# rsutormin/KmerGutsJava

Hardware: AMD Instinct MI355X
Metric: amino-acid residues/sec scanned (and hits/sec) on 1 Gbp synthetic, 1/2/4/8 MI355X (higher is better)
Workload: dtype int64; 1 GPU; 1 Gbp contig mix (0.5 kbp..1.024 Mbp, uniform ACGT) on 1 GPU, 6-frame translate + 8-mer lookup vs 1400303159-slot signature table (33.6 GB, load 0.50), -m 5 -g 200; total_bp_rank0=1000000000, contigs_rank0=6351, total_bp_all_ranks=1000000000, num_sigs=1400303159, residues_rank0=1999974596, residues_all_ranks=1999974596, hits_rank0=36744843, hits_all_ranks=36744843, calls_rank0=4, parallelism=contig shards x1, table replicated

## Files before the change

### kmergutsjava_amd/csrc/kg_host_plan.hpp

```cpp
#pragma once

namespace {


template <typename T, T V, T... Vs, typename F>
void dispatch(T x, F &&f)
{
    if constexpr (sizeof...(Vs) == 0) f(std::integral_constant<T, V>{});
    else if (x == V) f(std::integral_constant<T, V>{});
    else dispatch<T, Vs...>(x, f);
}

struct BatchPlan {
    std::vector<uint32_t> ibase;
    uint64_t nblocks = 0, windows = 0, residues = 0;
    uint64_t n_rows = 0, n_cont = 0;
    int64_t longest = 0;
};

template <bool AA>
int plan_batch(const int64_t *offsets, int64_t n_seqs, BatchPlan &b)
{
    constexpr uint32_t PER = AA ? 1 : 6;
    b.ibase.resize((size_t)n_seqs + 1);
    for (int64_t k = 0; k < n_seqs; k++) {
        int64_t L = offsets[k + 1] - offsets[k];
        if (L < 0) return fail(KG_ERR_ARG, "offsets must be non-decreasing");
        b.longest = std::max(b.longest, L);
        if (L > 0xFFFFFFF0ll) return fail(KG_ERR_LIMIT, "a single sequence longer than 2^32-16 characters");
        b.ibase[(size_t)k] = (uint32_t)b.nblocks;
        uint64_t nb;
        if (AA) {
            uint64_t nwin = L >= 9 ? (uint64_t)L - 8 : 0;
            b.windows += nwin;
            b.residues += (uint64_t)L;
            nb = (nwin + kg::kAaWinPerBlock - 1) / kg::kAaWinPerBlock;
        } else {
            uint64_t npos = L >= 24 ? (uint64_t)L - 23 : 0;
            b.windows += 2 * npos;
            for (int f = 0; f < 3; f++)
                if (L - f >= 3) b.residues += 2 * (uint64_t)((L - f) / 3);
            nb = (npos + kg::kDnaPosPerBlock - 1) / kg::kDnaPosPerBlock;
        }
        b.nblocks += nb;
        if (b.nblocks > 0x7FFFFFFFull / PER) return fail(KG_ERR_LIMIT, "batch too large: more than 2^31-1 window rows; split the batch");
    }
    b.ibase[(size_t)n_seqs] = (uint32_t)b.nblocks;
    if (b.windows > 0xFFFFFF00ull) return fail(KG_ERR_LIMIT, "batch too large: more than 2^32-256 windows; split the batch");
    b.n_rows = b.nblocks * PER;
    b.n_cont = (uint64_t)n_seqs * PER;
    return KG_OK;
}

uint64_t bucket_count(uint64_t limit, uint32_t shift) { return (limit + (1ull << shift) - 1) >> shift; }

struct PartPlan {
    bool applicable = false;
    uint32_t shift = 0, buckets = 0;
    uint32_t n_chunks = 0;
    std::vector<uint64_t> clo;
    std::vector<int64_t> cseq;
    uint64_t max_chunk = 0;
    uint32_t n_wg = 0, cap = 0;
    uint64_t n_regions = 0;
    uint32_t ovf_cap = 0;
    uint32_t gshift = 10, groups_stride = 0;
    size_t next_stride = 0;
    size_t scatter_lds = 0;
    bool use_bidx = false, part_counters = false, prog_index = false;
    uint32_t probe_grid = 0, index_grid = 0, verify_grid = 0, lowc_grid = 0, ovf_grid = 0, order_grid = 0;
    uint32_t scatter_prio = 0, index_prio = 0, verify_prio = 0, index_r = 1, probe_grab = 0;
    uint32_t flush_list = 0;
    uint64_t list_slack = 0, ucap = 0, ccap = 0;
    uint32_t n_os = 0;
    bool early_totals = false, place_staged = false, debug = false;
};

template <bool AA>
int plan_partition(const kg_table *t, const BatchPlan &b, bool progress, bool counters_req, PartPlan &pl)
{
    constexpr uint32_t PER = AA ? 1 : 6;
    const uint64_t nblocks = b.nblocks;
    uint32_t shift = env_knob("KG_PART_SHIFT", 21u, 4u, 31u);
    const uint64_t qmax = (uint64_t)KG_MAX_ENCODED / (uint64_t)t->num_sigs + 1;
    while (shift > 4 && qmax >= (1ull << (32 - shift))) shift--;
    while (bucket_count(t->limit, shift) > (uint64_t)kg::kMaxBuckets) shift++;
    while (kg::scatter_lds_bytes<AA>((uint32_t)bucket_count(t->limit, shift)) > 160u * 1024) shift++;
    const bool fits = shift < 32 && qmax < (1ull << (32 - shift)) && nblocks <= (1ull << 23) && t->m35 != 0 &&
                      t->limit < (1ull << 32) - 64;
    const uint32_t mode = env_u32("KG_PARTITION", 2u);
    const bool worth = t->limit >= (64ull << 20) && b.windows >= (1ull << 27);
    if (!(fits && nblocks > 0 && (mode == 1 || (mode == 2 && worth)))) return KG_OK;
    pl.shift = shift;
    pl.buckets = (uint32_t)bucket_count(t->limit, shift);

    constexpr uint32_t WIN = AA ? 64u : 384u;
    uint32_t want = env_u32("KG_PART_CHUNKS", 4u);
    if (want < 1) want = 1;
    if (want > kMaxChunks) want = kMaxChunks;
    if (getenv("KG_PART_MIN_CHUNK_BLOCKS")) {
        const uint64_t min_chunk = std::max(1u, env_u32("KG_PART_MIN_CHUNK_BLOCKS", 600000u));
        while (want > 1 && nblocks / want < min_chunk) want--;
    } else {
        const uint32_t by_size = nblocks < 450000 ? 1u : std::max(2u, (uint32_t)std::lround(std::sqrt((double)nblocks / 325000.0)));
        want = std::min(want, std::max(1u, by_size));
    }
    pl.clo.push_back(0); pl.cseq.push_back(0);
    std::vector<double> cum;
    if (const char *tp = getenv("KG_PART_TAPER")) {
        double acc = 0;
        for (const char *q = tp; *q;) {
            char *endp = nullptr;
            const double v = strtod(q, &endp);
            if (endp == q) break;
            acc += v; cum.push_back(acc);
            q = *endp == ',' ? endp + 1 : endp;
        }
        if (cum.size() >= 2 && cum.size() <= kMaxChunks && acc > 0) { for (auto &x : cum) x /= acc; want = (uint32_t)cum.size(); }
        else cum.clear();
    }
    for (uint32_t c = 1; c < want; c++) {
        const uint64_t target = cum.empty() ? nblocks * c / want : (uint64_t)((double)nblocks * cum[c - 1]);
        const auto it = std::lower_bound(b.ibase.begin(), b.ibase.end(), (uint32_t)target);
        const uint64_t cut = *it;
        if (cut > pl.clo.back() && cut < nblocks) { pl.clo.push_back(cut); pl.cseq.push_back((int64_t)(it - b.ibase.begin())); }
    }
    pl.clo.push_back(nblocks); pl.cseq.push_back((int64_t)b.ibase.size() - 1);
    pl.n_chunks = (uint32_t)pl.clo.size() - 1;
    for (uint32_t c = 0; c < pl.n_chunks; c++) pl.max_chunk = std::max(pl.max_chunk, pl.clo[c + 1] - pl.clo[c]);
    const uint64_t max_chunk = pl.max_chunk;
    const uint64_t chunk_blocks = (max_chunk + kg::kScatterWaves - 1) / kg::kScatterWaves * kg::kScatterWaves;
    const double max_frac = (double)max_chunk / (double)nblocks;
    uint32_t n_wg = env_knob("KG_PART_WGS", 256u, 1u, kMaxGrid);
    if ((uint64_t)n_wg * kg::kScatterWaves > chunk_blocks) n_wg = (uint32_t)((chunk_blocks + kg::kScatterWaves - 1) / kg::kScatterWaves);
    const uint64_t blocks_per_wg = ((chunk_blocks + (uint64_t)n_wg * kg::kScatterWaves - 1) / ((uint64_t)n_wg * kg::kScatterWaves)) * kg::kScatterWaves;
    const double mean = (double)blocks_per_wg * WIN / (double)pl.buckets * (env_u32("KG_PART_SLACK", 100u) / 100.0);
    const uint64_t cap64 = ((uint64_t)(mean + 6.0 * std::sqrt(mean) + 32.0) + 15) / 16 * 16;
    if (cap64 >= (1ull << 24) || (uint64_t)pl.buckets * n_wg >= (1ull << 24)) return KG_OK;
    pl.n_wg = n_wg;
    pl.cap = (uint32_t)cap64;
    pl.n_regions = (uint64_t)pl.buckets * n_wg;
    pl.ovf_cap = env_u32("KG_PART_OVF_GROUPS", (uint32_t)std::min<uint64_t>(1u << 23, std::max<uint64_t>(65536, pl.n_regions * pl.cap / 16 / 8)));
    while (pl.gshift < 12 && ((max_chunk * PER) >> pl.gshift) + 2 > 8192) pl.gshift++;
    pl.groups_stride = (uint32_t)(((max_chunk * PER) >> pl.gshift) + 2);
    if (pl.groups_stride > kg::kMaxGroups) return fail(KG_ERR_LIMIT, "a chunk of the batch holds more than 2^26 window rows");
    pl.next_stride = std::max<size_t>((size_t)pl.buckets + 8, 256);
    pl.use_bidx = t->d_bidx != nullptr && !counters_req && env_u32("KG_BIDX", 1u) != 0;
    pl.part_counters = (counters_req || progress) && !pl.use_bidx;
    pl.prog_index = progress && pl.use_bidx;
    pl.scatter_lds = kg::scatter_lds_bytes<AA>(pl.buckets);
    pl.flush_list = env_knob("KG_SCATTER_FLUSH_LIST", kg::scatter_flush_list_max<AA>(), 1u, kg::scatter_flush_list_max<AA>());
    pl.probe_grid = env_knob("KG_PROBE_GRID", 256u * 8u, 8u, kMaxGrid, 8u);
    pl.index_grid = env_knob("KG_INDEX_GRID", 256u * 4u, 8u, kMaxGrid, 8u);
    pl.scatter_prio = std::min(3u, env_u32("KG_SCATTER_PRIO", 1u));
    pl.index_prio = std::min(3u, env_u32("KG_INDEX_PRIO", 2u));
    pl.verify_prio = std::min(3u, env_u32("KG_VERIFY_PRIO", pl.n_chunks == 1 ? 2u : 0u));
    uint32_t index_r = env_u32("KG_INDEX_R", 0u);
    if (index_r == 0) index_r = mean * 0.7 >= 640.0 ? 1u : mean * 0.7 >= 320.0 ? 2u : 4u;
    if (index_r != 1 && index_r != 2) index_r = 4;
    while (index_r > 1 && (n_wg % index_r != 0 || kg::kIndexN % index_r != 0)) index_r /= 2;
    pl.index_r = index_r;
    pl.verify_grid = env_knob("KG_VERIFY_GRID", 256u * 2u, 1u, kMaxGrid);
    pl.lowc_grid = env_knob("KG_LOWC_GRID", 256u, 1u, kMaxGrid);
    pl.ovf_grid = env_knob("KG_OVF_GRID", 256u, 1u, kMaxGrid);
    pl.list_slack = (uint64_t)(std::max(std::max(pl.probe_grid, pl.index_grid), pl.verify_grid) + 64) * 4 * kg::kUChunk + 4096;
    pl.ucap = ((uint64_t)((double)b.windows * t->stage_ratio * max_frac) + pl.list_slack + kg::kUChunk - 1) / kg::kUChunk * kg::kUChunk;
    pl.ccap = ((uint64_t)((double)b.windows * (t->stage_ratio * 1.25 + 0.03) * max_frac) + pl.list_slack + kg::kUChunk - 1) /
              kg::kUChunk * kg::kUChunk;
    if (test_hook("KG_TEST_TINY_LISTS")) pl.ucap = pl.ccap = kg::kUChunk;
    const uint32_t grab_unit = 256u * (uint32_t)std::max(kg::kProbeN, kg::kIndexN);
    pl.probe_grab = env_knob("KG_PROBE_GRAB", pl.cap, grab_unit, 1u << 24, grab_unit);
    pl.n_os = pl.n_chunks < 2 ? 0u : std::min(env_u32("KG_ORDER_STREAMS", 0u), kMaxOrderStreams);
    pl.early_totals = pl.n_os == 0 && env_u32("KG_EARLY_TOTALS", 1u) != 0;
    pl.order_grid = env_knob("KG_ORDER_GRID", 256u * 3u, 1u, kMaxGrid);
    pl.place_staged = pl.gshift == 10 && env_u32("KG_PLACE_STAGED", 1u) != 0;
    pl.debug = getenv("KG_DEBUG") != nullptr;
    pl.applicable = true;
    return KG_OK;
}

struct DirectPlan {
    uint32_t scan_grid, stage_chunk;
    const uint32_t *d_hbits;
    uint32_t rpg;
    uint64_t stage_cap;
};

template <bool AA>
DirectPlan plan_direct(const kg_table *t, const BatchPlan &b, bool counters)
{
    DirectPlan pl;
    pl.scan_grid = env_knob("KG_SCAN_GRID", 256u * 8u, 1u, kMaxGrid);
    pl.stage_chunk = env_knob("KG_STAGE_CHUNK", 256u, 1u, 1u << 12);
    const uint32_t filter_mode = env_u32("KG_DIRECT_FILTER", 1u);
    pl.d_hbits = (counters || filter_mode == 0 || (filter_mode == 1 && t->limit <= (4ull << 20))) ? nullptr : t->d_hbits;
    pl.rpg = AA ? 1u : env_u32("KG_SCAN_RPG", pl.d_hbits ? 6u : 3u);
    if (pl.rpg != 1 && pl.rpg != 2 && pl.rpg != 3 && pl.rpg != 6) pl.rpg = 3;
    pl.stage_cap = (uint64_t)((double)b.windows * t->stage_ratio) + 4096 + (uint64_t)pl.scan_grid * kg::kWavesPerWG * pl.stage_chunk;
    if (pl.stage_cap > 0xFFFFFF00ull) pl.stage_cap = 0xFFFFFF00ull;
    if (test_hook("KG_TEST_TINY_LISTS")) pl.stage_cap = 256;
    return pl;
}

struct AggPlan {
    uint32_t pshift;
    bool pieces_on;
    uint32_t agg_pairs;
};

AggPlan plan_aggregate()
{
    AggPlan pl;
    pl.pshift = std::min(20u, std::max(6u, env_u32("KG_AGG_BLOCK_SHIFT", 9u)));
    pl.pieces_on = env_u32("KG_AGG_PIECES", 1u) != 0;
    pl.agg_pairs = env_u32("KG_AGG_PAIRS", 1u);
    return pl;
}

}
```

### kmergutsjava_amd/csrc/kg_partition.hpp

```cpp
#pragma once

#include "kg_device.hpp"

namespace kg {

constexpr int kMaxBuckets = 1024;
#ifndef KG_PROBE_N
#define KG_PROBE_N 4
#endif
#ifndef KG_SCATTER_WPE
#define KG_SCATTER_WPE 5
#endif
#ifndef KG_TAG_WPE
#define KG_TAG_WPE 8
#endif
#if KG_SCATTER_WPE
#define KG_SCATTER_REGS __attribute__((amdgpu_waves_per_eu(KG_SCATTER_WPE)))
#else
#define KG_SCATTER_REGS
#endif
#if KG_TAG_WPE
#define KG_TAG_REGS __attribute__((amdgpu_waves_per_eu(KG_TAG_WPE)))
#else
#define KG_TAG_REGS
// ... 229 lines not shown
                        lowc = true;
                        if (RG != ROWS) wave_sync();
                    }
                }
            }
        }
        n_valid += nv;
        uint32_t spins = 0;
        if (insert_prio) set_wave_prio(insert_prio);
        for (;;) {
            uint32_t at[RG], old[RG];
#pragma unroll
            for (int r = 0; r < RG; r++)
                at[r] = (pend & (1u << r)) ? atomicAdd(&cnt[bk[r]], 1u) : kGroup;
#pragma unroll
            for (int r = 0; r < RG; r++) {
                old[r] = 0;
                if (at[r] < kGroup) {
                    buf[(size_t)bk[r] * kGroup + at[r]] = e[r];
                    __builtin_amdgcn_fence(__ATOMIC_RELEASE, "wavefront");
                    old[r] = atomicAdd(&written[bk[r]], 1u);
                }
            }
            __builtin_amdgcn_fence(__ATOMIC_ACQUIRE, "wavefront");
#pragma unroll
            for (int r = 0; r < RG; r++) pend &= ~((uint32_t)(at[r] < kGroup) << r);
            uint32_t at_max = at[0];
#pragma unroll
            for (int r = 1; r < RG; r++) at_max = max(at_max, at[r]);
            uint32_t left = 0;
            auto list_rows = [&](auto again) -> uint32_t {
                uint32_t n = 0;
#pragma unroll
                for (int r = 0; r < RG; r++) {
                    const bool own = decltype(again)::value ? ((left >> r) & 1u) != 0 : (old[r] & 15u) == 15u;
                    const unsigned long long m = __ballot(own);
                    if (m) {
                        const uint32_t rank = __builtin_amdgcn_mbcnt_hi((uint32_t)(m >> 32), __builtin_amdgcn_mbcnt_lo((uint32_t)m, n));
                        if (own && rank < list_cap) {
                            const uint32_t g = decltype(again)::value ? (written[bk[r]] >> 4) - 1u : old[r] >> 4;
                            flist[rank] = (min(g, gcap) << 10) | bk[r];
                            if (decltype(again)::value) left &= ~(1u << r);
                        }
                        n += (uint32_t)__popcll(m);
                    }
                }
                return n;
            };
            uint32_t n_own = list_rows(std::false_type{});
            if (__builtin_expect(n_own > list_cap, 0)) {
                uint32_t k = 0;
#pragma unroll
                for (int r = 0; r < RG; r++) {
                    const bool own = (old[r] & 15u) == 15u;
                    const unsigned long long m = __ballot(own);
                    const uint32_t rank = __builtin_amdgcn_mbcnt_hi((uint32_t)(m >> 32), __builtin_amdgcn_mbcnt_lo((uint32_t)m, k));
                    if (own && rank >= list_cap) left |= 1u << r;
                    k += (uint32_t)__popcll(m);
                }
            }
            while (n_own) {
                const uint32_t n_list = min(n_own, list_cap);
                wave_sync();
                for (uint32_t p0 = 0; p0 < n_list; p0 += 8) {
                    const uint32_t want = p0 + ((uint32_t)lane >> 3), sub = (uint32_t)lane & 7u;
                    if (want < n_list) {
                        const uint32_t d = flist[want];
                        const uint32_t fb = d & (uint32_t)(kMaxBuckets - 1), g = d >> 10;
                        const ulonglong2 v = *reinterpret_cast<const ulonglong2 *>(buf + (size_t)fb * kGroup + 2 * sub);
                        __builtin_amdgcn_fence(__ATOMIC_RELEASE, "wavefront");
                        if (sub == 0) cnt[fb] = 0;
                        const bool full = g >= gcap;
                        if (!full) {
                            unsigned char *to = reinterpret_cast<unsigned char *>(ent) + (mul24_wide(__umul24(fb, n_wg) + w, cap) << 3);
                            store_entry_pair(reinterpret_cast<uint64_t *>(to + ((g << 7) | (sub << 4))), v);
                        }
                        if (__builtin_expect(__ballot(full) != 0, 0)) scatter_overflow_octets(cold, full, fb, v.x, v.y);
                    }
                }
                wave_sync();
                if (__builtin_expect(n_own <= list_cap, 1)) break;
                n_own = list_rows(std::true_type{});
            }
            if (!__ballot(pend != 0)) break;
            {
                const int rp = pend ? __builtin_ctz(pend) : 0;
                uint32_t pb = bk[0];
#pragma unroll
                for (int r = 1; r < RG; r++)
                    if (rp == r) pb = bk[r];
                for (uint32_t polls = 0; polls < 64; polls++) {
                    if (__ballot(pend != 0 && __hip_atomic_load(&cnt[pb], __ATOMIC_RELAXED, __HIP_MEMORY_SCOPE_WORKGROUP) < kGroup)) break;
                    __builtin_amdgcn_s_sleep(2);
                }
            }
            if (__builtin_expect(++spins > (1u << 20) || __ballot(at_max >= (1u << 28)), 0)) {
                scatter_protocol_failure(cold);
                break;
            }
        }
        if (insert_prio) set_wave_prio(0);
        }
    }
    __syncthreads();
    const uint32_t per_wave = (n_buckets + kScatterWaves - 1) / kScatterWaves;
    const uint32_t b_end = min((uint32_t)(wave + 1) * per_wave, n_buckets);
    for (uint32_t b0 = (uint32_t)wave * per_wave; b0 < b_end; b0 += 64) {
        const uint32_t b = b0 + (uint32_t)lane;
        const uint32_t wr = b < b_end ? written[b] : 0u;
        const uint32_t c = wr & 15u, g = wr >> 4;
        unsigned long long dst = kDstNone;
        bool to_ovf = false;
        if (c > 0) {
            for (uint32_t k = c; k < kGroup; k++) buf[(size_t)b * kGroup + k] = kEntInvalid;
            if (g < gcap) dst = ((uint64_t)b * n_wg + w) * cap + ((uint64_t)g << 4);
            else to_ovf = true;
        }
        const unsigned long long movf = __ballot(to_ovf);
        if (movf) dst = scatter_overflow_groups(cold, movf, to_ovf, b, dst);
        unsigned long long m = __ballot(dst != kDstNone);
        wave_sync();
        while (m) {
            int src_lane = -1;
            unsigned long long mm = m;
#pragma unroll
            for (int o = 0; o < 8; o++) {
                const int ln = mm ? __builtin_ctzll(mm) : -1;
                if (mm) mm &= mm - 1;
                if ((lane >> 3) == o) src_lane = ln;
            }
            m = mm;
            const int sl = src_lane < 0 ? 0 : src_lane;
            const uint32_t fb = (uint32_t)__shfl((int)b, sl);
            const unsigned long long to = __shfl(dst, sl);
            if (src_lane >= 0) {
                const uint32_t sub = (uint32_t)lane & 7u;
                const ulonglong2 v = *reinterpret_cast<const ulonglong2 *>(buf + (size_t)fb * kGroup + 2 * sub);
                if (__builtin_expect((to & kDstOvf) != 0, 0)) {
                    if (to != kDstDropped) scatter_store_overflow(cold, to, sub, v.x, v.y);
                } else {
                    store_entry_pair(ent + to + 2 * sub, v);
                }
            }
        }
    }
    for (uint32_t b = threadIdx.x; b < n_buckets; b += blockDim.x)
        fill[(uint64_t)b * n_wg + w] = min((written[b] + 15u) >> 4, gcap) << 4;
    for (int off = 32; off > 0; off >>= 1) n_valid += __shfl_down(n_valid, off);
    unsigned long long *ctr = cold->ctr;
    if (lane == 0 && n_valid) atomicAdd(&ctr[0], (unsigned long long)n_valid);
    if constexpr (SHORT) flush_ran_off(ran_off, ctr, lane);
}

constexpr int kLowcWaves = 4;
template <bool AA>
__global__ __launch_bounds__(64 * kLowcWaves) void lowc_blocks_kernel(
    const uint8_t *__restrict__ seq, const BlockDesc *__restrict__ blocks, const uint32_t *__restrict__ lowc_cursor,
    const uint32_t *__restrict__ lowc_blocks, uint64_t limit, uint32_t num_sigs, uint32_t m35, uint32_t shift, uint32_t n_regions,
    uint32_t cap, uint64_t *__restrict__ ent, uint32_t *__restrict__ fill, uint32_t *ovf_cursor, uint32_t ovf_cap,
    uint32_t *__restrict__ ovf_bucket, uint64_t *__restrict__ ovf_ent, unsigned long long *ctr, Progress *prog)
{
    constexpr int ROWS = AA ? 1 : 6;
    __shared__ typename WaveLds<AA>::type lds[kLowcWaves];
    __shared__ typename WaveLds<AA>::tables enc_tables;
    const int lane = threadIdx.x & 63, wave = threadIdx.x >> 6;
    typename WaveLds<AA>::type &l = lds[wave];
    const uint32_t n_list = *lowc_cursor;
    if (n_list == 0) return;
    encode_init<AA>(enc_tables, threadIdx.x, blockDim.x);
    __syncthreads();
    const uint32_t limit32 = limit < 0xFFFFFFFFull ? (uint32_t)limit : 0xFFFFFFFFu;
    unsigned long long n_valid = 0;
    bool ran_off = false;
    uint32_t pool_at = 0, pool_end = 0;
    auto pool_flush = [&]() {
        for (uint32_t g = pool_at + ((uint32_t)lane >> 4); g < pool_end && g < ovf_cap; g += 4) {
            if ((lane & 15) == 0) ovf_bucket[g] = 0;
            ovf_ent[(uint64_t)g * kGroup + ((uint32_t)lane & 15u)] = kEntInvalid;
        }
        pool_at = pool_end;
    };
    auto ovf_groups = [&](uint32_t lead, uint32_t ng) -> uint64_t * {
        if (pool_end - pool_at < ng) {
            pool_flush();
            const uint32_t want = ng > 32u ? ng : 32u;
            uint32_t g0 = 0;
            if (lane == 0) g0 = atomicAdd(ovf_cursor, want);
            g0 = (uint32_t)__builtin_amdgcn_readfirstlane((int)g0);
            pool_at = g0; pool_end = g0 + want;
        }
        const uint32_t g = pool_at;
        pool_at += ng;
        if (g + ng > ovf_cap) return nullptr;
        if ((uint32_t)lane < ng) ovf_bucket[g + lane] = lead;
        return ovf_ent + (uint64_t)g * kGroup;
    };
    for (uint32_t i = blockIdx.x * kLowcWaves + (uint32_t)wave; i < n_list; i += gridDim.x * kLowcWaves) {
        const uint32_t it = (uint32_t)__builtin_amdgcn_readfirstlane((int)lowc_blocks[i]);
        const BlockDesc bd = blocks[it];
        encode_block<AA>(l, enc_tables, seq, bd, lane);
        const uint32_t region_w = it % n_regions;
        for (int r = 0; r < ROWS; r++) {
            uint32_t hi, lo, q;
            bool valid = row_halves<AA>(l, r, lane, bd, &hi, &lo);
            const uint32_t slot = split_fast(hi, lo, num_sigs, m35, &q);
            if (valid) n_valid++;
            if (valid && slot >= limit32) { ran_off = true; if (prog) progress_note_beyond(prog, slot); }
            bool pend = valid && slot < limit32;
            const uint32_t bkt = slot >> shift;
            const uint64_t e = ((uint64_t)window_key<AA>(bd, it, r, lane) << 32) | ((q << shift) | (slot & ((1u << shift) - 1u)));
            for (int pass = 0; pass < 4; pass++) {
                const unsigned long long mp = __ballot(pend);
                if (__popcll(mp) < 16) break;
                const uint32_t lead = (uint32_t)__builtin_amdgcn_readlane((int)bkt, __builtin_ctzll(mp));
                const bool mine = pend && bkt == lead;
                const unsigned long long same = __ballot(mine);
                const uint32_t n = (uint32_t)__popcll(same);
                if (n < 8) break;
                const uint32_t rank = (uint32_t)__popcll(same & ((1ull << lane) - 1ull));
                const uint64_t region = (uint64_t)lead * n_regions + region_w;
                uint32_t rel = cap;
                if (lane == 0 && *const_cast<volatile uint32_t *>(&fill[region]) < cap) rel = atomicAdd(&fill[region], n);
                rel = (uint32_t)__builtin_amdgcn_readfirstlane((int)rel);
                if (rel + n <= cap) {
                    if (mine) ent[region * cap + rel + rank] = e;
                } else {
                    if (rel < cap && (uint32_t)lane < cap - rel) ent[region * cap + rel + lane] = kEntInvalid;
                    const uint32_t npad = (n + kGroup - 1) & ~(kGroup - 1);
                    uint64_t *dst = ovf_groups(lead, npad / kGroup);
                    if (dst) {
                        if (mine) dst[rank] = e;
                        if ((uint32_t)lane < npad - n) dst[n + lane] = kEntInvalid;
                    }
                }
                if (mine) pend = false;
            }
            if (pend) {
                const uint64_t region = (uint64_t)bkt * n_regions + region_w;
                const uint32_t rel = atomicAdd(&fill[region], 1u);
                if (rel < cap) { ent[region * cap + rel] = e; pend = false; }
            }
            for (;;) {
                const unsigned long long mp = __ballot(pend);
                if (!mp) break;
                const uint32_t lead = (uint32_t)__builtin_amdgcn_readlane((int)bkt, __builtin_ctzll(mp));
                const bool mine = pend && bkt == lead;
                const unsigned long long same = __ballot(mine);
                const uint32_t n = (uint32_t)__popcll(same);
                const uint32_t npad = (n + kGroup - 1) & ~(kGroup - 1);
                const uint32_t rank = (uint32_t)__popcll(same & ((1ull << lane) - 1ull));
                uint64_t *dst = ovf_groups(lead, npad / kGroup);
                if (dst) {
                    if (mine) dst[rank] = e;
                    if ((uint32_t)lane < npad - n) dst[n + lane] = kEntInvalid;
                }
                if (mine) pend = false;
            }
        }
        wave_sync();
    }
    pool_flush();
    for (int off = 32; off > 0; off >>= 1) n_valid += __shfl_down(n_valid, off);
    if (lane == 0 && n_valid) atomicAdd(&ctr[0], n_valid);
    flush_ran_off(ran_off, ctr, lane);
}

struct UListState { unsigned long long base; uint32_t used; bool have; };

template <bool AA, int N, bool COUNTERS>
__device__ __forceinline__ void probe_entries(const TableView &tab, uint32_t b, uint32_t shift, const uint64_t (&e)[N],
                                              kg_hit *__restrict__ ulist, uint32_t *__restrict__ chunk_used,
                                              unsigned long long *cursor, uint64_t ulist_cap, UListState &u,
                                              unsigned long long &ctr_slots, bool &ran_off, int lane, Progress *prog)
{
    uint64_t val[N], slot[N];
    bool valid[N];
    uint32_t id[N], fp[N];
#pragma unroll
    for (int k = 0; k < N; k++) {
        valid[k] = e[k] != kEntInvalid;
        const uint32_t low = (uint32_t)e[k];
        id[k] = (uint32_t)(e[k] >> 32);
        slot[k] = ((uint64_t)b << shift) | (low & ((1u << shift) - 1u));
        val[k] = (uint64_t)(low >> shift) * tab.num_sigs + slot[k];
        fp[k] = tag_qs(low >> shift, slot[k]);
    }
    Payload pay[N];
    unsigned long long ctr_dummy = 0;
    uint32_t fslot[N];
#pragma unroll
    for (int k = 0; k < N; k++) fslot[k] = 0;
    const uint32_t foundm = probe_n<N, COUNTERS>(tab, val, slot, fp, valid, pay, ctr_dummy, ctr_slots, ran_off, COUNTERS ? prog : nullptr,
                                                 COUNTERS ? fslot : nullptr);
    uint32_t cnt[N], rank[N], total = 0;
#pragma unroll
    for (int k = 0; k < N; k++) {
        const bool f = (foundm >> k) & 1u;
        const unsigned long long m = __ballot(f);
        cnt[k] = (uint32_t)__popcll(m);
        rank[k] = (uint32_t)__popcll(m & ((1ull << lane) - 1ull));
        total += cnt[k];
    }
    if (total) {
        if (u.used + total > kUChunk) {
            if (lane == 0 && u.have && u.base + kUChunk <= ulist_cap) chunk_used[u.base / kUChunk] = u.used;
            unsigned long long nb = 0;
            if (lane == 0) nb = atomicAdd(cursor, (unsigned long long)kUChunk);
            nb = ((unsigned long long)__builtin_amdgcn_readfirstlane((uint32_t)(nb >> 32)) << 32) |
                 (unsigned long long)__builtin_amdgcn_readfirstlane((uint32_t)nb);
            u.base = nb; u.used = 0; u.have = true;
        }
        if (u.base + kUChunk <= ulist_cap) {
            uint32_t at = u.used;
#pragma unroll
            for (int k = 0; k < N; k++) {
                if ((foundm >> k) & 1u) {
                    kg_hit h;
                    h.container = id[k];
                    h.from0InProt = (int32_t)fslot[k];
                    h.oI = pay[k].oI; h.avgOffFromEnd = pay[k].avg; h.fI = pay[k].fI; h.functionWt = pay[k].wt;
                    ulist[u.base + at + rank[k]] = h;
                }
                at += cnt[k];
            }
        }
        u.used += total;
    }
}

struct CandRec { uint32_t home, quo, id, walked; };
constexpr uint32_t kWalkOn = 0x80000000u;
constexpr uint32_t kScanOn = 0x40000000u;
constexpr uint32_t kWalkedMask = 0x3FFFFFFFu;
static_assert(sizeof(CandRec) == 16, "CandRec must be 16 bytes");

__device__ __forceinline__ unsigned long long chunk_reserve(UListState &u, uint32_t total, uint32_t *__restrict__ chunk_used,
                                                            unsigned long long *cursor, uint64_t cap, int lane)
{
    if (u.used + total > kUChunk) {
        if (lane == 0 && u.have && u.base + kUChunk <= cap) chunk_used[u.base / kUChunk] = u.used;
        unsigned long long nb = 0;
        if (lane == 0) nb = atomicAdd(cursor, (unsigned long long)kUChunk);
        nb = ((unsigned long long)__builtin_amdgcn_readfirstlane((uint32_t)(nb >> 32)) << 32) |
             (unsigned long long)__builtin_amdgcn_readfirstlane((uint32_t)nb);
        u.base = nb; u.used = 0; u.have = true;
    }
    const unsigned long long at = u.base + u.used;
    u.used += total;
    return u.base + kUChunk <= cap ? at : ~0ull;
}

__device__ __forceinline__ void chunk_finish(const UListState &u, uint32_t *__restrict__ chunk_used, uint64_t cap, int lane)
{
    if (lane == 0 && u.have && u.base + kUChunk <= cap) chunk_used[u.base / kUChunk] = u.used;
}

template <bool COUNTERS>
__global__ __launch_bounds__(256) KG_TAG_REGS void bucket_tag_kernel(
    const uint8_t *__restrict__ tags, uint64_t limit, uint64_t num_sigs, const uint64_t *__restrict__ ent,
    const uint32_t *__restrict__ fill, uint32_t n_regions, uint32_t cap, uint32_t n_buckets, uint32_t shift,
    uint32_t grab ,
    uint32_t *next_region ,
    CandRec *__restrict__ cand, uint32_t *__restrict__ cand_used, unsigned long long *cand_cursor, uint64_t cand_cap,
// ... 109 lines not shown
        const CandRec out = stage[(uint32_t)lane < sfill ? lane : 0];
        const unsigned long long at = chunk_reserve(u, sfill, cand_used, cand_cursor, cand_cap, lane);
        if (at != ~0ull && (uint32_t)lane < sfill) stream_store16(cand + at + (uint32_t)lane, &out);
    }
    chunk_finish(u, cand_used, cand_cap, lane);
    flush_ran_off(ran_off, ctr, lane);
    if (COUNTERS) {
        for (int off = 32; off > 0; off >>= 1) ctr_slots += __shfl_down(ctr_slots, off);
        if (lane == 0) atomicAdd(&ctr[1], ctr_slots);
    }
}

template <int N, int R, bool EXACT, bool PROG = false>
__global__ __launch_bounds__(256) KG_TAG_REGS void bucket_index_kernel(
    const uint8_t *__restrict__ bidx, uint32_t tail_start,
    const uint64_t *__restrict__ ent, const uint32_t *__restrict__ fill, uint32_t n_regions , uint32_t cap, uint32_t n_buckets,
    uint32_t shift, uint32_t grab ,
    uint32_t *next_region ,
    CandRec *__restrict__ cand, uint32_t *__restrict__ cand_used, unsigned long long *cand_cursor, uint64_t cand_cap,
    unsigned long long *ctr, uint32_t prio , Progress *prog )
{
    static_assert(N % R == 0, "R must divide N");
    constexpr int PER = N / R;
    __shared__ uint32_t s_region;
    __shared__ uint32_t s_lut[256];
    __shared__ __attribute__((aligned(16))) CandRec s_stage[4][kStageFlush + 64];
    CandRec *stage = s_stage[__builtin_amdgcn_readfirstlane((int)(threadIdx.x >> 6))];
    uint32_t sfill = 0;
    const int lane = threadIdx.x & 63;
    bool ran_off = false;
    UListState u;
    u.base = 0; u.used = kUChunk; u.have = false;
    s_lut[threadIdx.x] = bidx_decode(threadIdx.x);
    if (prio) set_wave_prio(prio);

    const uint32_t kGrab = grab;
    const uint32_t grabs_per_region = (cap + kGrab - 1) / kGrab;
    const uint32_t n_grabs = (n_regions / R) * grabs_per_region;
    const uint32_t xg = blockIdx.x & 7u;
    const uint32_t n_tickets = xg < n_buckets ? ((n_buckets - xg + 7u) / 8u) * n_grabs : 0u;
    constexpr uint32_t all_walk = EXACT ? 0u : kBidxInexact;
    for (;;) {
        __syncthreads();
        if (threadIdx.x == 0) s_region = atomicAdd(&next_region[xg * 32u], 1u);
        __syncthreads();
        const uint32_t tk = s_region;
        if (tk >= n_tickets) break;
        const uint32_t b = xg + 8u * (tk / n_grabs), g = tk % n_grabs;
        const uint32_t w = (g / grabs_per_region) * R, g0 = (g % grabs_per_region) * kGrab;
        uint32_t fraw[R], n[R], nmax = cap;
#pragma unroll
        for (int r = 0; r < R; r++) { fraw[r] = fill[(uint64_t)b * n_regions + w + r]; n[r] = cap; }
        const uint64_t *src = ent + ((uint64_t)b * n_regions + w) * cap;
        const uint32_t smask = (1u << shift) - 1u, bbase = b << shift;
        uint32_t d_lo = 0, d_hi = 0, pmin = ~0u, pmax1 = 0;
        if (PROG) {
            const uint64_t s0 = (uint64_t)b << shift, s1 = (((uint64_t)b + 1) << shift) - 1;
#pragma unroll
            for (int k = 1; k <= 10; k++) { d_lo += prog->lo[k] <= s0 ? 1u : 0u; d_hi += prog->lo[k] <= s1 ? 1u : 0u; }
        }
        for (uint32_t c0 = g0; c0 < nmax && c0 < g0 + kGrab; c0 += 256u * PER) {
            uint64_t ev[N];
#pragma unroll
            for (int k = 0; k < N; k++) {
                const int r = k / PER;
                const uint32_t i = c0 + (uint32_t)(k % PER) * 256u + threadIdx.x;
                ev[k] = i < n[r] ? __builtin_nontemporal_load(src + (uint64_t)r * cap + i) : kEntInvalid;
            }
            if (c0 == g0) {
                nmax = 0;
#pragma unroll
                for (int r = 0; r < R; r++) {
                    uint32_t f = fraw[r];
                    asm volatile("; fill first used here" : "+s"(f));
                    n[r] = min(f, cap);
                    nmax = max(nmax, n[r]);
                }
            }
            uint32_t code[N], vmask = 0;
#pragma unroll
            for (int k = 0; k < N; k++) {
                if (c0 + (uint32_t)(k % PER) * 256u + threadIdx.x >= n[k / PER]) ev[k] = kEntInvalid;
                code[k] = 0;
                if (ev[k] != kEntInvalid) {
                    vmask |= 1u << k;
                    code[k] = bidx[bbase | ((uint32_t)ev[k] & smask)];
                }
            }
            uint32_t candm = 0, walkm = 0, wd[N];
#pragma unroll
            for (int k = 0; k < N; k++) wd[k] = s_lut[code[k]];
#pragma unroll
            for (int k = 0; k < N; k++) {
                const uint32_t q = (uint32_t)ev[k] >> shift;
                const uint32_t c = EXACT ? q : q % kBidxClasses;
                const uint32_t listed = (wd[k] >> c) & 1u;
                candm |= listed << k;
                walkm |= (listed & ((wd[k] | all_walk) >> 31)) << k;
                ran_off = ran_off || (((vmask >> k) & 1u) && !listed && (bbase | ((uint32_t)ev[k] & smask)) >= tail_start);
            }
            if (PROG) {
                if (d_lo == d_hi) {
#pragma unroll
                    for (int k = 0; k < N; k++) {
                        const uint32_t h = bbase | ((uint32_t)ev[k] & smask);
                        if ((vmask >> k) & 1u) pmin = min(pmin, h);
                        if (((vmask & ~candm) >> k) & 1u) pmax1 = max(pmax1, h + 1u);
                    }
                } else {
                    for (int k = 0; k < N; k++)
                        if ((vmask >> k) & 1u) progress_note_home(prog, d_lo, d_hi, bbase | ((uint32_t)ev[k] & smask), (candm >> k) & 1u);
                }
            }
#pragma unroll
            for (int k = 0; k < N; k++) {
                const unsigned long long m = __ballot((candm >> k) & 1u);
                if (!m) continue;
                if ((candm >> k) & 1u) {
                    CandRec c;
                    c.home = bbase | ((uint32_t)ev[k] & smask); c.quo = (uint32_t)ev[k] >> shift;
                    c.id = (uint32_t)(ev[k] >> 32); c.walked = ((walkm >> k) & 1u) ? kWalkOn : kScanOn;
                    stage[sfill + (uint32_t)__popcll(m & ((1ull << lane) - 1ull))] = c;
                }
                sfill += (uint32_t)__popcll(m);
                while (sfill >= kStageFlush) {
                    wave_sync();
                    const unsigned long long at = chunk_reserve(u, kStageFlush, cand_used, cand_cursor, cand_cap, lane);
                    if ((uint32_t)lane < kStageFlush) {
                        const ulonglong2 out = *reinterpret_cast<const ulonglong2 *>(stage + lane);
                        if (at != ~0ull) stream_store16(cand + at + (uint32_t)lane, &out);
                    }
                    sfill -= kStageFlush;
                    wave_sync();
                    if ((uint32_t)lane < sfill) {
                        const ulonglong2 rest = *reinterpret_cast<const ulonglong2 *>(stage + kStageFlush + lane);
                        *reinterpret_cast<ulonglong2 *>(stage + lane) = rest;
                    }
                    wave_sync();
                }
            }
        }
        if (PROG && d_lo == d_hi) progress_note_homes(prog, d_lo, pmin, pmax1);
    }
    if (sfill) {
        wave_sync();
        const CandRec out = stage[(uint32_t)lane < sfill ? lane : 0];
        const unsigned long long at = chunk_reserve(u, sfill, cand_used, cand_cursor, cand_cap, lane);
        if (at != ~0ull && (uint32_t)lane < sfill) stream_store16(cand + at + (uint32_t)lane, &out);
    }
    chunk_finish(u, cand_used, cand_cap, lane);
    flush_ran_off(ran_off, ctr, lane);
}

template <bool AA, bool COUNTERS, bool PROG = false>
__global__ __launch_bounds__(256) void verify_kernel(
    const uint8_t *__restrict__ entries, const uint8_t *__restrict__ tags, uint64_t limit, uint64_t num_sigs, uint64_t magic,
    const CandRec *__restrict__ cand, const uint32_t *__restrict__ cand_used, const unsigned long long *cand_cursor,
    uint64_t cand_cap, kg_hit *__restrict__ ulist, uint32_t *__restrict__ chunk_used, unsigned long long *cursor,
    uint64_t ulist_cap, unsigned long long *ctr, Progress *prog ,
    uint32_t prio )
{
    const int lane = threadIdx.x & 63;
    const uint32_t wave_global = __builtin_amdgcn_readfirstlane(blockIdx.x * 4 + (threadIdx.x >> 6));
    const uint32_t n_waves = gridDim.x * 4;
    if (prio) set_wave_prio(prio);
    TableView tab;
    tab.entries = entries; tab.tags = tags; tab.limit = limit; tab.num_sigs = num_sigs; tab.magic = magic; tab.m35 = 0;
    const unsigned long long cur = *cand_cursor;
    const uint32_t n_chunks = (uint32_t)((cur < cand_cap ? cur : cand_cap) / kUChunk);
    unsigned long long ctr_slots = 0;
    bool ran_off = false;
    UListState u;
    u.base = 0; u.used = kUChunk; u.have = false;
    for (uint32_t c = wave_global; c < n_chunks; c += n_waves) {
        const uint32_t used = cand_used[c];
        for (uint32_t k0 = 0; k0 < used; k0 += 64) {
            const bool act = k0 + (uint32_t)lane < used;
            CandRec r;
            r.home = 0; r.quo = 0; r.id = 0; r.walked = 0;
            if (act) {
                const kg_u32x4 cv = __builtin_nontemporal_load(reinterpret_cast<const kg_u32x4 *>(cand + (uint64_t)c * kUChunk + k0 + lane));
                r.home = cv.x; r.quo = cv.y; r.id = cv.z; r.walked = cv.w;
            }
            const uint64_t quo = r.quo, home = r.home;
            const uint64_t val = quo * num_sigs + home;
            uint64_t s = home + (r.walked & kWalkedMask);
            bool found = false;
            Entry e;
            e.key = 0; e.oI = e.avg = e.fI = 0; e.wt = 0.f;
            if (act && (r.walked & kScanOn)) {
#if KG_SCAN_FULL
                if (s < limit) {
                    const uint64_t s1 = s + 1 < limit ? s + 1 : s, s2 = s + 2 < limit ? s + 2 : s;
                    const Entry e0 = load_entry(tab, s);
                    const uint2 k1 = *reinterpret_cast<const uint2 *>(tab.entries + s1 * 24);
                    const uint2 k2 = *reinterpret_cast<const uint2 *>(tab.entries + s2 * 24);
                    const uint32_t vlo = (uint32_t)val, vhi = (uint32_t)(val >> 32);
                    if (e0.key == (int64_t)val) { found = true; e = e0; }
                    else if (s + 1 < limit && k1.x == vlo && k1.y == vhi) { found = true; s += 1; e = load_entry(tab, s); }
                    else if (s + 2 < limit && k2.x == vlo && k2.y == vhi) { found = true; s += 2; e = load_entry(tab, s); }
                    else s += 3;
                }
#endif
                while (!found) {
                    if (s >= limit) { s = limit; ran_off = true; break; }
                    const uint64_t s1 = s + 1 < limit ? s + 1 : s, s2 = s + 2 < limit ? s + 2 : s;
                    const uint2 k0 = *reinterpret_cast<const uint2 *>(tab.entries + s * 24);
                    const uint2 k1 = *reinterpret_cast<const uint2 *>(tab.entries + s1 * 24);
                    const uint2 k2 = *reinterpret_cast<const uint2 *>(tab.entries + s2 * 24);
                    const uint32_t vlo = (uint32_t)val, vhi = (uint32_t)(val >> 32);
                    if (k0.x == vlo && k0.y == vhi) found = true;
                    else if (s + 1 < limit && k1.x == vlo && k1.y == vhi) { found = true; s += 1; }
                    else if (s + 2 < limit && k2.x == vlo && k2.y == vhi) { found = true; s += 2; }
                    if (found) { e = load_entry(tab, s); break; }
                    s += 3;
                }
                if (COUNTERS) {
                    ctr_slots += (s < limit ? s + 1 : limit) - home;
                    if (prog) progress_note_walk(prog, home, s, limit);
                } else if (PROG) {
                    progress_note_walk(prog, home, s, limit);
                }
            } else if (act) {
                if (!(r.walked & kWalkOn)) {
                    e = load_entry(tab, s);
                    found = e.key == (int64_t)val;
                    if (!found) s += 1;
                }
                if (!found) {
                    const uint32_t f = tag_qs(quo, home);
                    for (;;) {
                        if (s >= limit) { s = limit; ran_off = true; break; }
                        const Tags16 x = load_tags(tab.tags + s);
                        bool emp;
                        const int i = first_stop(x, f, &emp);
                        if (i == 16) { s += 16; continue; }
                        s += (uint64_t)i;
                        if (emp) { if (s >= limit) ran_off = true; break; }
                        e = load_entry(tab, s);
                        if (e.key == (int64_t)val) { found = true; break; }
                        s += 1;
                    }
                }
                if (COUNTERS) {
                    ctr_slots += (s < limit ? s + 1 : limit) - home;
                    if (prog) progress_note_walk(prog, home, s, limit);
                } else if (PROG) {
                    progress_note_walk(prog, home, s, limit);
                }
            }
            const unsigned long long m = __ballot(found);
            const uint32_t total = (uint32_t)__popcll(m);
            if (total) {
                const unsigned long long at = chunk_reserve(u, total, chunk_used, cursor, ulist_cap, lane);
                if (at != ~0ull && found) {
                    kg_hit h;
                    h.container = r.id;
                    h.from0InProt = (int32_t)(uint32_t)s;
                    h.oI = e.oI; h.avgOffFromEnd = e.avg; h.fI = e.fI; h.functionWt = e.wt;
                    stream_store_hit(ulist + at + (uint32_t)__popcll(m & ((1ull << lane) - 1ull)), h);
                }
            }
        }
    }
    chunk_finish(u, chunk_used, ulist_cap, lane);
    flush_ran_off(ran_off, ctr, lane);
    if (COUNTERS) {
        for (int off = 32; off > 0; off >>= 1) ctr_slots += __shfl_down(ctr_slots, off);
        if (lane == 0) atomicAdd(&ctr[1], ctr_slots);
    }
}

template <bool AA, bool COUNTERS, bool PROG = false>
__global__ __launch_bounds__(256) void overflow_probe_kernel(
    const uint8_t *__restrict__ entries, const uint8_t *__restrict__ tags, uint64_t limit, uint64_t num_sigs, uint64_t magic,
    const uint32_t *__restrict__ ovf_bucket, const uint64_t *__restrict__ ovf_ent, const uint32_t *__restrict__ ovf_cursor,
    uint32_t ovf_cap, uint32_t shift, kg_hit *__restrict__ ulist, uint32_t *__restrict__ chunk_used, unsigned long long *cursor, uint64_t ulist_cap,
    unsigned long long *ctr, Progress *prog)
{
    const int lane = threadIdx.x & 63;
    const uint32_t wave_global = __builtin_amdgcn_readfirstlane(blockIdx.x * 4 + (threadIdx.x >> 6));
    const uint32_t n_waves = gridDim.x * 4;
    TableView tab;
    tab.entries = entries; tab.tags = tags; tab.limit = limit; tab.num_sigs = num_sigs; tab.magic = magic; tab.m35 = 0;
    unsigned long long ctr_slots = 0;
    bool ran_off = false;
    UListState u;
    u.base = 0; u.used = kUChunk; u.have = false;
    const uint32_t n_groups = min(*ovf_cursor, ovf_cap);
    for (uint32_t g = wave_global; g < n_groups; g += n_waves) {
        const uint32_t b = ovf_bucket[g];
        uint64_t e[1];
        e[0] = lane < (int)kGroup ? ovf_ent[(uint64_t)g * kGroup + lane] : kEntInvalid;
        probe_entries<AA, 1, COUNTERS || PROG>(tab, b, shift, e, ulist, chunk_used, cursor, ulist_cap, u, ctr_slots, ran_off, lane, prog);
    }
    if (lane == 0 && u.have && u.base + kUChunk <= ulist_cap) chunk_used[u.base / kUChunk] = u.used;
    flush_ran_off(ran_off, ctr, lane);
    if (COUNTERS) {
        for (int off = 32; off > 0; off >>= 1) ctr_slots += __shfl_down(ctr_slots, off);
        if (lane == 0) atomicAdd(&ctr[1], ctr_slots);
    }
}

__global__ void chunk_base_kernel(const uint64_t *chunk_total, uint64_t *base, uint64_t *grand_total)
{
    const uint64_t b = base[0] + *chunk_total;
    base[1] = b;
    if (grand_total) *grand_total = b;
}

}
```

Baseline: 132.5 billion residues/s.

## Shrink lowc kernel to one wave per block and narrow verify indices to 32-bit

```diff
diff --git a/kmergutsjava_amd/csrc/kg_host_plan.hpp b/kmergutsjava_amd/csrc/kg_host_plan.hpp
--- a/kmergutsjava_amd/csrc/kg_host_plan.hpp
+++ b/kmergutsjava_amd/csrc/kg_host_plan.hpp
@@ -161,7 +161,7 @@
     while (index_r > 1 && (n_wg % index_r != 0 || kg::kIndexN % index_r != 0)) index_r /= 2;
     pl.index_r = index_r;
     pl.verify_grid = env_knob("KG_VERIFY_GRID", 256u * 2u, 1u, kMaxGrid);
-    pl.lowc_grid = env_knob("KG_LOWC_GRID", 256u, 1u, kMaxGrid);
+    pl.lowc_grid = env_knob("KG_LOWC_GRID", 256u * 4u, 1u, kMaxGrid);
     pl.ovf_grid = env_knob("KG_OVF_GRID", 256u, 1u, kMaxGrid);
     pl.list_slack = (uint64_t)(std::max(std::max(pl.probe_grid, pl.index_grid), pl.verify_grid) + 64) * 4 * kg::kUChunk + 4096;
     pl.ucap = ((uint64_t)((double)b.windows * t->stage_ratio * max_frac) + pl.list_slack + kg::kUChunk - 1) / kg::kUChunk * kg::kUChunk;
diff --git a/kmergutsjava_amd/csrc/kg_partition.hpp b/kmergutsjava_amd/csrc/kg_partition.hpp
--- a/kmergutsjava_amd/csrc/kg_partition.hpp
+++ b/kmergutsjava_amd/csrc/kg_partition.hpp
@@ -405,7 +405,7 @@
     if constexpr (SHORT) flush_ran_off(ran_off, ctr, lane);
 }
 
-constexpr int kLowcWaves = 4;
+constexpr int kLowcWaves = 1;
 template <bool AA>
 __global__ __launch_bounds__(64 * kLowcWaves) void lowc_blocks_kernel(
     const uint8_t *__restrict__ seq, const BlockDesc *__restrict__ blocks, const uint32_t *__restrict__ lowc_cursor,
@@ -420,7 +420,12 @@
     typename WaveLds<AA>::type &l = lds[wave];
     const uint32_t n_list = *lowc_cursor;
     if (n_list == 0) return;
-    encode_init<AA>(enc_tables, threadIdx.x, blockDim.x);
+#pragma unroll 1
+    for (uint32_t k = 0; k < 256; k += 64 * kLowcWaves) {
+        uint32_t tid = threadIdx.x + k;
+        asm volatile("" : "+v"(tid));
+        encode_init<AA>(enc_tables, tid, 256u);
+    }
     __syncthreads();
     const uint32_t limit32 = limit < 0xFFFFFFFFull ? (uint32_t)limit : 0xFFFFFFFFu;
     unsigned long long n_valid = 0;
@@ -451,9 +456,14 @@
     for (uint32_t i = blockIdx.x * kLowcWaves + (uint32_t)wave; i < n_list; i += gridDim.x * kLowcWaves) {
         const uint32_t it = (uint32_t)__builtin_amdgcn_readfirstlane((int)lowc_blocks[i]);
         const BlockDesc bd = blocks[it];
-        encode_block<AA>(l, enc_tables, seq, bd, lane);
+        int lane_b = lane;
+        asm volatile("" : "+v"(lane_b));
+        encode_block<AA>(l, enc_tables, seq, bd, lane_b);
         const uint32_t region_w = it % n_regions;
+#pragma unroll 1
         for (int r = 0; r < ROWS; r++) {
+            int lane = lane_b;
+            asm volatile("" : "+v"(lane));
             uint32_t hi, lo, q;
             bool valid = row_halves<AA>(l, r, lane, bd, &hi, &lo);
             const uint32_t slot = split_fast(hi, lo, num_sigs, m35, &q);
@@ -462,6 +472,7 @@
             bool pend = valid && slot < limit32;
             const uint32_t bkt = slot >> shift;
             const uint64_t e = ((uint64_t)window_key<AA>(bd, it, r, lane) << 32) | ((q << shift) | (slot & ((1u << shift) - 1u)));
+#pragma unroll 1
             for (int pass = 0; pass < 4; pass++) {
                 const unsigned long long mp = __ballot(pend);
                 if (__popcll(mp) < 16) break;
@@ -877,9 +888,14 @@
     flush_ran_off(ran_off, ctr, lane);
 }
 
+__device__ __forceinline__ const uint2 *record_at(const uint8_t *__restrict__ entries, uint32_t slot)
+{
+    return reinterpret_cast<const uint2 *>(entries + (uint64_t)slot * 24u);
+}
+
 template <bool AA, bool COUNTERS, bool PROG = false>
 __global__ __launch_bounds__(256) void verify_kernel(
-    const uint8_t *__restrict__ entries, const uint8_t *__restrict__ tags, uint64_t limit, uint64_t num_sigs, uint64_t magic,
+    const uint8_t *__restrict__ entries, const uint8_t *__restrict__ tags, uint64_t limit64, uint64_t num_sigs, uint64_t magic,
     const CandRec *__restrict__ cand, const uint32_t *__restrict__ cand_used, const unsigned long long *cand_cursor,
     uint64_t cand_cap, kg_hit *__restrict__ ulist, uint32_t *__restrict__ chunk_used, unsigned long long *cursor,
     uint64_t ulist_cap, unsigned long long *ctr, Progress *prog ,
@@ -889,8 +905,7 @@
     const uint32_t wave_global = __builtin_amdgcn_readfirstlane(blockIdx.x * 4 + (threadIdx.x >> 6));
     const uint32_t n_waves = gridDim.x * 4;
     if (prio) set_wave_prio(prio);
-    TableView tab;
-    tab.entries = entries; tab.tags = tags; tab.limit = limit; tab.num_sigs = num_sigs; tab.magic = magic; tab.m35 = 0;
+    const uint32_t limit = (uint32_t)limit64, n_sigs = (uint32_t)num_sigs;
     const unsigned long long cur = *cand_cursor;
     const uint32_t n_chunks = (uint32_t)((cur < cand_cap ? cur : cand_cap) / kUChunk);
     unsigned long long ctr_slots = 0;
@@ -907,71 +922,77 @@
                 const kg_u32x4 cv = __builtin_nontemporal_load(reinterpret_cast<const kg_u32x4 *>(cand + (uint64_t)c * kUChunk + k0 + lane));
                 r.home = cv.x; r.quo = cv.y; r.id = cv.z; r.walked = cv.w;
             }
-            const uint64_t quo = r.quo, home = r.home;
-            const uint64_t val = quo * num_sigs + home;
-            uint64_t s = home + (r.walked & kWalkedMask);
+            const uint64_t val = (uint64_t)r.quo * n_sigs + r.home;
+            const uint32_t vlo = (uint32_t)val, vhi = (uint32_t)(val >> 32);
+            uint32_t s = r.home + (r.walked & kWalkedMask);
             bool found = false;
-            Entry e;
-            e.key = 0; e.oI = e.avg = e.fI = 0; e.wt = 0.f;
+            uint2 pa = make_uint2(0u, 0u), pb = make_uint2(0u, 0u);
             if (act && (r.walked & kScanOn)) {
 #if KG_SCAN_FULL
                 if (s < limit) {
-                    const uint64_t s1 = s + 1 < limit ? s + 1 : s, s2 = s + 2 < limit ? s + 2 : s;
-                    const Entry e0 = load_entry(tab, s);
-                    const uint2 k1 = *reinterpret_cast<const uint2 *>(tab.entries + s1 * 24);
-                    const uint2 k2 = *reinterpret_cast<const uint2 *>(tab.entries + s2 * 24);
-                    const uint32_t vlo = (uint32_t)val, vhi = (uint32_t)(val >> 32);
-                    if (e0.key == (int64_t)val) { found = true; e = e0; }
-                    else if (s + 1 < limit && k1.x == vlo && k1.y == vhi) { found = true; s += 1; e = load_entry(tab, s); }
-                    else if (s + 2 < limit && k2.x == vlo && k2.y == vhi) { found = true; s += 2; e = load_entry(tab, s); }
-                    else s += 3;
+                    const uint32_t s1 = s + 1 < limit ? s + 1 : s, s2 = s + 2 < limit ? s + 2 : s;
+                    const uint2 *p0 = record_at(entries, s);
+                    const uint2 k0r = p0[0];
+                    pa = p0[1]; pb = p0[2];
+                    const uint2 k1 = *record_at(entries, s1);
+                    const uint2 k2 = *record_at(entries, s2);
+                    uint32_t d = 3;
+                    if (k0r.x == vlo && k0r.y == vhi) d = 0;
+                    else if (s + 1 < limit && k1.x == vlo && k1.y == vhi) d = 1;
+                    else if (s + 2 < limit && k2.x == vlo && k2.y == vhi) d = 2;
+                    s += d;
+                    found = d < 3;
+                    if (d == 1 || d == 2) { const uint2 *p = record_at(entries, s); pa = p[1]; pb = p[2]; }
                 }
 #endif
                 while (!found) {
                     if (s >= limit) { s = limit; ran_off = true; break; }
-                    const uint64_t s1 = s + 1 < limit ? s + 1 : s, s2 = s + 2 < limit ? s + 2 : s;
-                    const uint2 k0 = *reinterpret_cast<const uint2 *>(tab.entries + s * 24);
-                    const uint2 k1 = *reinterpret_cast<const uint2 *>(tab.entries + s1 * 24);
-                    const uint2 k2 = *reinterpret_cast<const uint2 *>(tab.entries + s2 * 24);
-                    const uint32_t vlo = (uint32_t)val, vhi = (uint32_t)(val >> 32);
-                    if (k0.x == vlo && k0.y == vhi) found = true;
+                    const uint32_t s1 = s + 1 < limit ? s + 1 : s, s2 = s + 2 < limit ? s + 2 : s;
+                    const uint2 k0r = *record_at(entries, s);
+                    const uint2 k1 = *record_at(entries, s1);
+                    const uint2 k2 = *record_at(entries, s2);
+                    if (k0r.x == vlo && k0r.y == vhi) found = true;
                     else if (s + 1 < limit && k1.x == vlo && k1.y == vhi) { found = true; s += 1; }
                     else if (s + 2 < limit && k2.x == vlo && k2.y == vhi) { found = true; s += 2; }
-                    if (found) { e = load_entry(tab, s); break; }
+                    if (found) { const uint2 *p = record_at(entries, s); pa = p[1]; pb = p[2]; break; }
                     s += 3;
                 }
                 if (COUNTERS) {
-                    ctr_slots += (s < limit ? s + 1 : limit) - home;
-                    if (prog) progress_note_walk(prog, home, s, limit);
+                    ctr_slots += (s < limit ? s + 1 : limit) - r.home;
+                    if (prog) progress_note_walk(prog, r.home, s, limit);
                 } else if (PROG) {
-                    progress_note_walk(prog, home, s, limit);
+                    progress_note_walk(prog, r.home, s, limit);
                 }
             } else if (act) {
                 if (!(r.walked & kWalkOn)) {
-                    e = load_entry(tab, s);
-                    found = e.key == (int64_t)val;
+                    const uint2 *p = record_at(entries, s);
+                    const uint2 k = p[0];
+                    pa = p[1]; pb = p[2];
+                    found = k.x == vlo && k.y == vhi;
                     if (!found) s += 1;
                 }
                 if (!found) {
-                    const uint32_t f = tag_qs(quo, home);
+                    const uint32_t f = tag_qs(r.quo, r.home);
                     for (;;) {
                         if (s >= limit) { s = limit; ran_off = true; break; }
-                        const Tags16 x = load_tags(tab.tags + s);
+                        const Tags16 x = load_tags(tags + s);
                         bool emp;
                         const int i = first_stop(x, f, &emp);
                         if (i == 16) { s += 16; continue; }
-                        s += (uint64_t)i;
+                        s += (uint32_t)i;
                         if (emp) { if (s >= limit) ran_off = true; break; }
-                        e = load_entry(tab, s);
-                        if (e.key == (int64_t)val) { found = true; break; }
+                        const uint2 *p = record_at(entries, s);
+                        const uint2 k = p[0];
+                        pa = p[1]; pb = p[2];
+                        if (k.x == vlo && k.y == vhi) { found = true; break; }
                         s += 1;
                     }
                 }
                 if (COUNTERS) {
-                    ctr_slots += (s < limit ? s + 1 : limit) - home;
-                    if (prog) progress_note_walk(prog, home, s, limit);
+                    ctr_slots += (s < limit ? s + 1 : limit) - r.home;
+                    if (prog) progress_note_walk(prog, r.home, s, limit);
                 } else if (PROG) {
-                    progress_note_walk(prog, home, s, limit);
+                    progress_note_walk(prog, r.home, s, limit);
                 }
             }
             const unsigned long long m = __ballot(found);
@@ -981,8 +1002,8 @@
                 if (at != ~0ull && found) {
                     kg_hit h;
                     h.container = r.id;
-                    h.from0InProt = (int32_t)(uint32_t)s;
-                    h.oI = e.oI; h.avgOffFromEnd = e.avg; h.fI = e.fI; h.functionWt = e.wt;
+                    h.from0InProt = (int32_t)s;
+                    h.oI = (int32_t)pa.x; h.avgOffFromEnd = (int32_t)pa.y; h.fI = (int32_t)pb.x; h.functionWt = __uint_as_float(pb.y);
                     stream_store_hit(ulist + at + (uint32_t)__popcll(m & ((1ull << lane) - 1ull)), h);
                 }
             }
```

After: 130.9 billion residues/s. 1.2% lower.
